# MohamedAbou-Taleb/Iterative-Linear-Quadratic-Regulator

Hardware: AMD Instinct MI355X
Metric: iLQR iterations/sec (batch=4096, T=200, n=4 m=1); backward-pass HBM GB/s (higher is better)
Workload: dtype f32

## Files before the change

### iterative-linear-quadratic-regulator_amd/csrc/backward_fused16.hpp

```cpp
#pragma once

namespace ilqr {

template <typename T, int TPW, bool PK> struct FusedCfg;
template <> struct FusedCfg<float, 16, false> { static constexpr int P = 8, RU = 8; };
#ifndef ILQR_PK_RU
#define ILQR_PK_RU 5
#endif
#ifndef ILQR_PK_PAD
#define ILQR_PK_PAD 0
#endif
template <> struct FusedCfg<float, 16, true> { static constexpr int P = 4, RU = ILQR_PK_RU; };
template <> struct FusedCfg<double, 16, false> { static constexpr int P = 4, RU = 4; };
template <> struct FusedCfg<float, 4, false> { static constexpr int P = 3, RU = 4; };
template <> struct FusedCfg<double, 4, false> { static constexpr int P = 3, RU = 3; };

template <int NU> constexpr int fused_tl() { return NU == 2 ? 68 : 52; }
template <bool PK, int NU> constexpr int fused_unit_scalars() { return (PK ? 128 : 64) * fused_tl<NU>() + (PK ? 64 * ILQR_PK_PAD : 0); }
template <typename T, int TPW, bool PK, int NU> constexpr int fused_ru() { return (PK && NU == 2 && FusedCfg<T, TPW, PK>::RU > 4) ? 4 : FusedCfg<T, TPW, PK>::RU; }
template <typename T, int TPW, bool PK, int NU = 1> constexpr int fused_lds_bytes() {
    return fused_ru<T, TPW, PK, NU>() * fused_unit_scalars<PK, NU>() * (int)sizeof(T) + (fused_ru<T, TPW, PK, NU>() + 4 + 32 + 4) * 4;
}
static_assert(fused_lds_bytes<float, 16, true, 1>() <= 160 * 1024 && fused_lds_bytes<float, 16, true, 2>() <= 160 * 1024 &&
              fused_lds_bytes<float, 16, false, 2>() <= 160 * 1024 && fused_lds_bytes<double, 16, false, 2>() <= 160 * 1024, "LDS ring exceeds a CU");
template <typename T, int TPW, bool PK> constexpr int fused_threads() { return 64 * (TPW / 4 + FusedCfg<T, TPW, PK>::P); }

template <typename T, int NU> struct FusedStep;
template <> struct FusedStep<float, 1> {
    using Tile = TileQ;
    static ILQR_DEV void load(Tile& t, const float* tp, int i, int j, int l16) {
        const float4 s = *reinterpret_cast<const float4*>(tp + 4 * j);
        const float4 v = *reinterpret_cast<const float4*>(tp + 32 + 4 * j);
        t.skj[0] = s.x; t.skj[1] = s.y; t.skj[2] = s.z; t.skj[3] = s.w;
        t.vj[0] = v.x; t.vj[1] = v.y; t.vj[2] = v.z; t.vj[3] = v.w;
        t.a = tp[l16];
        t.lxx = tp[16 + l16];
        t.c = tp[32 + l16];
    }
    static ILQR_DEV void step(const Tile& c, const LaneConst<float>& lc, int i, int j, float& V, float& vx, float& out, bool& pd) {
        RawTileQ none;
        const i32x4 srd = {0, 0, 0, 0};
        const TileOffsets off = {0, 0, 0};
        float Kj, kff;
        tile16_step_f32<false>(c, lc, V, vx, Kj, kff, pd, none, srd, off, 0);
        out = (i == 0) ? Kj : kff;
    }
    static ILQR_DEV void step_box(const Tile& c, const LaneConst<float>& lc, int i, int j, float u, float lo, float hi,
                                  float& V, float& vx, float& out, bool& pd) {
        RawTileQ none;
        const i32x4 srd = {0, 0, 0, 0};
        const TileOffsets off = {0, 0, 0};
        float Kj, kff;
        tile16_step_f32<false, true>(c, lc, V, vx, Kj, kff, pd, none, srd, off, 0, u, lo, hi);
        out = (i == 0) ? Kj : kff;
    }
};
template <> struct FusedStep<double, 1> {
    using Tile = Tile16<double>;
    static ILQR_DEV void load(Tile& t, const double* tp, int i, int j, int l16) { tile16_load_lds(t, tp, i, j, l16); }
    static ILQR_DEV void step(const Tile& c, const LaneConst<double>& lc, int i, int j, double& V, double& vx, double& out, bool& pd) {
        double Kj, kff;
        tile16_step<double, false>(c, lc, 0.0, V, vx, Kj, kff, pd);
        out = (i == 0) ? Kj : kff;
    }
    static ILQR_DEV void step_box(const Tile& c, const LaneConst<double>& lc, int i, int j, double u, double lo, double hi,
                                  double& V, double& vx, double& out, bool& pd) {
        double Kj, kff;
        tile16_step<double, false, true>(c, lc, 0.0, V, vx, Kj, kff, pd, u, lo, hi);
        out = (i == 0) ? Kj : kff;
    }
};
template <> struct FusedStep<float, 2> {
    using Tile = TileQ2;
    static ILQR_DEV void load(Tile& t, const float* tp, int i, int j, int l16) { tileq2_load_lds(t, tp, i, j, l16); }
    static ILQR_DEV void step(const Tile& c, const LaneConst<float>& lc, int i, int j, float& V, float& vx, float& out, bool& pd) {
        const GainSel sel = GainSel::of(i, j);
        tile16m2_step_f32(c, lc, sel, V, vx, out, pd);
    }
};
template <typename T> struct FusedStep<T, 2> {
    using Tile = Tile16M2<T>;
    using V4 = typename Vec4<T>::type;
    static ILQR_DEV void load(Tile& t, const T* tp, int i, int j, int l16) {
        const V4 si = *reinterpret_cast<const V4*>(tp + 4 * i);
        const V4 sj = *reinterpret_cast<const V4*>(tp + 4 * j);
        const V4 g0 = *reinterpret_cast<const V4*>(tp + 32 + 8 * j);
        const V4 g1 = *reinterpret_cast<const V4*>(tp + 36 + 8 * j);
        t.ski[0] = si.x; t.ski[1] = si.y; t.ski[2] = si.z; t.ski[3] = si.w;
        t.skj[0] = sj.x; t.skj[1] = sj.y; t.skj[2] = sj.z; t.skj[3] = sj.w;
        t.gj[0] = g0.x; t.gj[1] = g0.y; t.gj[2] = g0.z; t.gj[3] = g0.w;
        t.gj[4] = g1.x; t.gj[5] = g1.y; t.gj[6] = g1.z; t.gj[7] = g1.w;
        const T* gi = tp + 32 + 8 * i;
        t.gi[0] = gi[0]; t.gi[1] = gi[1]; t.gi[3] = gi[3]; t.gi[4] = gi[4];
        t.lxx = tp[16 + l16];
    }
    static ILQR_DEV void step(const Tile& c, const LaneConst<T>& lc, int i, int j, T& V, T& vx, T& out, bool& pd) {
        T K0, K1, k0, k1;
        tile16m2_step<T, false>(c, lc.m0, lc.m1, T(0), V, vx, K0, K1, k0, k1, pd);
        out = (i == 0) ? K0 : ((i == 1) ? K1 : ((j == 0) ? k0 : k1));
    }
};

ILQR_DEV void compiler_fence() { asm volatile("" ::: "memory"); }
ILQR_DEV int lds_peek(const int* p) { return __hip_atomic_load(p, __ATOMIC_RELAXED, __HIP_MEMORY_SCOPE_WORKGROUP); }
ILQR_DEV void lds_poke(int* p, int v) { __hip_atomic_store(p, v, __ATOMIC_RELAXED, __HIP_MEMORY_SCOPE_WORKGROUP); }

template <typename T, typename Dyn, int INTEG, int TPW, bool PK, bool BOX, bool HET> struct FusedRoles {
    static constexpr int NX = Dyn::NX, NU = Dyn::NU;
    static_assert(!BOX || (NU == 1 && fused_tl<1>() > kTile16), "control limits: n_u = 1, u_t in the tile's padding");
    static_assert((NU == 1 && NX >= 2 && NX <= 4) || (NX == 4 && NU == 2), "the fused sweep serves the DPP tiles: n_u = 1, or (4, 2)");
    static_assert(TPW == 16 || TPW == 4, "16 or 4 trajectories per workgroup");
    static_assert(!PK || (sizeof(T) == 4 && TPW == 16 && INTEG != ILQR_INT_BACKWARD_EULER), "pair producers: fp32, 16-trajectory workgroups, explicit integrators");
    using Cfg = FusedCfg<T, TPW, PK>;
    static constexpr int P = Cfg::P, RU = fused_ru<T, TPW, PK, NU>(), TL = fused_tl<NU>();
    static constexpr int NV = (NU == 2 ? kTile16M2 : kTile16) / 4;
    static constexpr int NSW = TPW / 4;
    static constexpr int UT = PK ? 128 : 64;
    static constexpr int US = UT / TPW;
    static constexpr int UNIT = fused_unit_scalars<PK, NU>();
    static constexpr int PS = 2 * TL + ILQR_PK_PAD;
    static constexpr int R = gain_record(NX, NU);
    using PL = ParamLayout<Dyn::NSYS, NX, NU>;
    using V4 = typename Vec4<T>::type;
    static ILQR_DEV constexpr int tile_off(int r, int tl) { return PK ? ((r / 2) * TPW + tl) * PS + (r % 2) * TL : (r * TPW + tl) * TL; }
    static ILQR_DEV constexpr int step_off(int r) { return PK ? (r / 2) * TPW * PS + (r % 2) * TL : r * TPW * TL; }

    struct Lds {
        T* ring;
        int* ready;
        int* done;
        int* s_slot;
        int* s_stat;
    };
    static ILQR_DEV Lds carve(unsigned char* base) {
        Lds L;
        L.ring = reinterpret_cast<T*>(base);
        L.ready = reinterpret_cast<int*>(base + (size_t)RU * UNIT * sizeof(T));
        L.done = L.ready + RU;
        L.s_slot = L.done + 4;
        L.s_stat = L.s_slot + 16;
        return L;
    }

    static ILQR_DEV void head(const KArgs<T>& a, const Lds& L, int b0, int lane, bool do_select, bool count) {
        bool still = false;
        if (lane < 16) {
            const int b = b0 + lane;
            int slot = 0, st = -1;
            if (lane < TPW && b < a.B) {
                if (do_select) {
                    still = select_candidates(a, b, true, slot, st);
                } else {
                    st = a.status[b];
                    slot = a.cur_slot[b];
                }
                a.cur_slot[b] = traj_active(st) ? 0 : slot;
            }
            L.s_slot[lane] = slot;
            L.s_stat[lane] = st;
        } else if (lane < 16 + RU + 4) {
            L.ready[lane - 16] = 0;
        }
        if (do_select && count) {
            const unsigned long long m = __ballot(still);
            if (lane == 0 && m) atomicAdd(&a.counters[a.counter_idx], (int)__popcll(m));
            if (blockIdx.x == 0 && lane == 0) a.counters[(a.counter_idx + 1) % kCounterRing] = 0;
        }
    }
    static ILQR_DEV bool any_active(const Lds& L) {
        bool any = false;
#pragma unroll
        for (int q = 0; q < 16; ++q) any = any || traj_active(L.s_stat[q]);
        return any;
    }

    static ILQR_DEV void sweep(const KArgs<T>& a, const Lds& L, int b0, int wave, int lane, ClockProbe& cp) {
        const size_t B = a.B;
        const int N = a.N;
        const int tid = threadIdx.x;
        (void)tid;
        __builtin_amdgcn_s_setprio(2);
        const int l16 = lane & 15, i = l16 >> 2, j = l16 & 3;
        const int tl = 4 * wave + (lane >> 4);
        const int gidx = b0 + tl;
        const bool valid = gidx < a.B;
        const int b = valid ? gidx : a.B - 1;
        const int st = L.s_stat[tl];
        const bool act = valid && traj_active(st);
        const int slot = act ? L.s_slot[tl] : 0;
        T ph[HET ? PL::TOTAL : 1];
        if constexpr (HET) {
#pragma unroll
            for (int q = 0; q < PL::TOTAL; ++q) ph[q] = a.params[q];
            load_row<PL::Q>(ph, a.rows, B, b);
        }
        const T* __restrict__ pp = HET ? ph : a.params;
        T xN[NX];
        vec_load<T, NX>(a.X + vec_at(B, N + 1, NX, slot, N, b), xN);
        if (act && slot != 0 && l16 == 0) vec_store<T, NX>(a.X + vec_at(B, N + 1, NX, 0, N, b), xN);
        T V = T(0), vx = T(0);
        {
            T g[NX], H[NX][NX];
            Cost<T, Dyn>::l_f_x(pp, xN, g);
            Cost<T, Dyn>::l_f_xx(pp, xN, H);
#pragma unroll
            for (int ii = 0; ii < NX; ++ii) {
                if (j == ii) vx = g[ii];
#pragma unroll
                for (int jj = 0; jj < NX; ++jj)
                    if (i == ii && j == jj) V = H[ii][jj];
            }
        }
        const unsigned gain_bytes = (unsigned)((size_t)N * B * R * sizeof(T));
        const __amdgpu_buffer_rsrc_t rgain = make_rsrc(a.gains, gain_bytes);
        const int rstride = (int)(B * R * sizeof(T));
        constexpr bool DROP = sizeof(T) == 4 || ILQR_DROP_ALL;
        const bool storer = act && (NU == 1 ? ((i == 0 && j < NX) || l16 == 4) : (i < 2 || (i == 2 && j < 2)));
        const int rec_slot = NU == 1 ? (i == 0 ? j : NX) : (i < 2 ? 4 * i + j : 8 + j);
        const int rec_off = (storer || !DROP) ? (int)((b * R + rec_slot) * sizeof(T)) : 0x7ffffff0;
        LaneConst<T> lc;
        lc.m0 = T(j == 0);
        lc.m1 = T(j == 1);
        lc.tr_byte = 4 * ((lane & 48) | (j << 2) | i);
        bool all_pd = true;
        using FS = FusedStep<T, NU>;
        const T blo = BOX ? a.u_lo[0] : T(0), bhi = BOX ? a.u_hi[0] : T(0);
        typename FS::Tile tq[2];
        T uq[2] = {T(0), T(0)};
        auto load = [&](int q, const T* tp) {
            FS::load(tq[q], tp, i, j, l16);
            if constexpr (BOX) uq[q] = tp[kTile16];
        };
        int goff = (N - 1) * rstride;
        auto unit_base = [&](int k) -> const T* { return L.ring + (size_t)(k % RU) * UNIT + tile_off(0, tl); };
        constexpr auto step_off = [](int r) { return PK ? (r / 2) * TPW * PS + (r % 2) * TL : r * TPW * TL; };
        auto one_step = [&](int q) {
            T out;
            bool pd;
            if constexpr (BOX) FS::step_box(tq[q], lc, i, j, uq[q], blo, bhi, V, vx, out, pd);
            else FS::step(tq[q], lc, i, j, V, vx, out, pd);
            all_pd = all_pd && pd;
            if (DROP || storer) buf_store1(rgain, rec_off, uniform(goff), out);
            goff -= rstride;
        };
#ifdef ILQR_FUSED_STAMPS
        const long long st_t0 = __builtin_readcyclecounter();
        long long st_spin = 0;
#endif
        while (lds_peek(&L.ready[0]) < 1) __builtin_amdgcn_s_sleep(1);
        compiler_fence();
#ifdef ILQR_FUSED_STAMPS
        const long long st_first = __builtin_readcyclecounter();
#endif
        load(0, unit_base(0));
        const int n_full = N / US, rem = N % US;
        for (int k = 0; k < n_full; ++k) {
            const T* ub = unit_base(k);
            const bool more = (k + 1) * US < N;
            int flag = 0;
#pragma unroll
            for (int r = 0; r < US; ++r) {
                if (r == US - 2 && more) flag = lds_peek(&L.ready[(k + 1) % RU]);
                if (r < US - 1) {
                    load((r + 1) & 1, ub + step_off(r + 1));
                } else if (more) {
#ifdef ILQR_FUSED_STAMPS
                    const long long w0 = __builtin_readcyclecounter();
#endif
                    while (flag < k + 2) {
                        __builtin_amdgcn_s_sleep(1);
                        flag = lds_peek(&L.ready[(k + 1) % RU]);
                    }
                    compiler_fence();
#ifdef ILQR_FUSED_STAMPS
                    st_spin += __builtin_readcyclecounter() - w0;
#endif
                    load(0, unit_base(k + 1));
                }
                one_step(r & 1);
            }
            compiler_fence();
            if (lane == 0) lds_poke(&L.done[wave], k + 1);
        }
        if (rem) {
            const T* ub = unit_base(n_full);
#pragma unroll
            for (int r = 0; r < US - 1; ++r) {
                if (r < rem) {
                    if (r + 1 < rem) load((r + 1) & 1, ub + step_off(r + 1));
                    one_step(r & 1);
                }
            }
        }
#ifdef ILQR_FUSED_STAMPS
        if (a.probe && blockIdx.x == 7 && tid == 0) {
            a.probe[5] = st_first - st_t0;
            a.probe[6] = st_spin;
            a.probe[7] = __builtin_readcyclecounter() - st_first;
        }
#endif
        cp.stop(a.probe, 0);
        if (act && l16 == 0 && !all_pd) a.status[b] = st | ILQR_TRAJ_FLAG_NON_PD;
    }

    static ILQR_DEV void produce(const KArgs<T>& a_, const Lds& L, int b0, int pw, int lane) {
        struct { int B; T dt; T* X; T* U; const T* params; const T* rows; } a = {a_.B, a_.dt, a_.X, a_.U, a_.params, a_.rows};
        const size_t B = a.B;
        const int N = a_.N;
        const int n_units = (N + US - 1) / US;
        if constexpr (PK) {
        using T2 = pair_f32;
        using Dyn2 = typename Dyn::template rebind<T2>;
        const int tl = lane % TPW, r2 = lane / TPW;
        const int gidx = b0 + tl;
        const bool valid = gidx < a.B;
        const int b = valid ? gidx : a.B - 1;
        const bool actb = valid && traj_active(L.s_stat[tl]);
        const int slot = actb ? L.s_slot[tl] : 0;
        const bool move = actb && slot != 0;
        T pl[PL::TOTAL];
#pragma unroll
        for (int q = 0; q < PL::TOTAL; ++q) pl[q] = a.params[q];
        if constexpr (HET) load_row<PL::Q>(pl, a.rows, B, b);
        const SplatParams p{pl};
        const T2 dt2 = a.dt;
        for (int k = pw; k < n_units; k += P) {
            const int ta = N - 1 - k * US - 2 * r2, tb = ta - 1;
            const bool ina = ta >= 0, inb = tb >= 0;
            const int tta = ina ? ta : 0, ttb = inb ? tb : 0;
            T xa[NX], ua[NU], xb[NX], ub[NU];
            vec_load<T, NX>(a.X + vec_at(B, N + 1, NX, slot, tta, b), xa);
            vec_load<T, NU>(a.U + vec_at(B, N, NU, slot, tta, b), ua);
            vec_load<T, NX>(a.X + vec_at(B, N + 1, NX, slot, ttb, b), xb);
            vec_load<T, NU>(a.U + vec_at(B, N, NU, slot, ttb, b), ub);
            if (move && ina) {
                vec_store<T, NX>(a.X + vec_at(B, N + 1, NX, 0, tta, b), xa);
                vec_store<T, NU>(a.U + vec_at(B, N, NU, 0, tta, b), ua);
            }
            if (move && inb) {
                vec_store<T, NX>(a.X + vec_at(B, N + 1, NX, 0, ttb, b), xb);
                vec_store<T, NU>(a.U + vec_at(B, N, NU, 0, ttb, b), ub);
            }
            T2 x[NX], u[NU], xn[NX], fx[NX][NX], fu[NX][NU];
#pragma unroll
            for (int q = 0; q < NX; ++q) { x[q].x = xa[q]; x[q].y = xb[q]; }
#pragma unroll
            for (int q = 0; q < NU; ++q) { u[q].x = ua[q]; u[q].y = ub[q]; }
            Stepper<T2, Dyn2>::step_jac(INTEG, p, dt2, x, u, xn, fx, fu);
            T2 gxn[NX], gu1[NU], lxxn[NX][NX], luxn[NU][NX], luu[NU][NU];
            Cost<T2, Dyn2>::grad(p, dt2, x, u, gxn, gu1);
            Cost<T2, Dyn2>::hess(p, dt2, x, u, lxxn, luxn, luu);
            V4 tile_a[NV], tile_b[NV];
            tile16_fill<T, NX, NU>([](T2 v) { return v.x; }, fx, fu, gxn, gu1, lxxn, luxn, luu, tile_a);
            tile16_fill<T, NX, NU>([](T2 v) { return v.y; }, fx, fu, gxn, gu1, lxxn, luxn, luu, tile_b);
            if (k >= RU) {
                const int need = k - RU + 1;
                auto slowest = [&]() {
                    int m = lds_peek(&L.done[0]);
#pragma unroll
                    for (int q = 1; q < NSW; ++q) m = min(m, lds_peek(&L.done[q]));
                    return m;
                };
                while (slowest() < need) __builtin_amdgcn_s_sleep(2);
            }
            compiler_fence();
            V4* dst = reinterpret_cast<V4*>(L.ring + (size_t)(k % RU) * UNIT + tile_off(2 * r2, tl));
            if (ina) {
#pragma unroll
                for (int q = 0; q < NV; ++q) dst[q] = tile_a[q];
            }
            if (inb) {
#pragma unroll
                for (int q = 0; q < NV; ++q) dst[TL / 4 + q] = tile_b[q];
            }
            if constexpr (BOX) {
                T* dt_ = reinterpret_cast<T*>(dst);
                if (ina) dt_[kTile16] = ua[0];
                if (inb) dt_[TL + kTile16] = ub[0];
            }
            compiler_fence();
            if (lane == 0) lds_poke(&L.ready[k % RU], k + 1);
        }
        } else {
        const int tl = lane % TPW, r = lane / TPW;
        const int gidx = b0 + tl;
        const bool valid = gidx < a.B;
        const int b = valid ? gidx : a.B - 1;
        const bool actb = valid && traj_active(L.s_stat[tl]);
        const int slot = actb ? L.s_slot[tl] : 0;
        const bool move = actb && slot != 0;
        T p[PL::TOTAL];
#pragma unroll
        for (int q = 0; q < PL::TOTAL; ++q) p[q] = a.params[q];
        if constexpr (HET) load_row<PL::Q>(p, a.rows, B, b);
        for (int k = pw; k < n_units; k += P) {
            const int t = N - 1 - k * US - r;
            const bool inr = t >= 0;
            const int tt = inr ? t : 0;
            T x[NX], u[NU];
            vec_load<T, NX>(a.X + vec_at(B, N + 1, NX, slot, tt, b), x);
            vec_load<T, NU>(a.U + vec_at(B, N, NU, slot, tt, b), u);
            if (move && inr) {
                vec_store<T, NX>(a.X + vec_at(B, N + 1, NX, 0, tt, b), x);
                vec_store<T, NU>(a.U + vec_at(B, N, NU, 0, tt, b), u);
            }
            T xn[NX], fx[NX][NX], fu[NX][NU];
            Stepper<T, Dyn>::step_jac(INTEG, p, a.dt, x, u, xn, fx, fu);
            V4 tile[NV];
            tile16_pack<T, Dyn>(p, a.dt, x, u, fx, fu, tile);
            if (k >= RU) {
                const int need = k - RU + 1;
                auto slowest = [&]() {
                    int m = lds_peek(&L.done[0]);
#pragma unroll
                    for (int q = 1; q < NSW; ++q) m = min(m, lds_peek(&L.done[q]));
                    return m;
                };
                while (slowest() < need) __builtin_amdgcn_s_sleep(2);
            }
            compiler_fence();
            if (inr) {
                constexpr int NQ = NV * (int)sizeof(V4) / 16;
                vec_u4 w[NQ];
                __builtin_memcpy(w, tile, sizeof(V4) * NV);
                vec_u4* dst = reinterpret_cast<vec_u4*>(L.ring + (size_t)(k % RU) * UNIT + tile_off(r, tl));
#pragma unroll
                for (int q = 0; q < NQ; ++q) dst[q] = w[q];
                if constexpr (BOX) reinterpret_cast<T*>(dst)[kTile16] = u[0];
            }
            compiler_fence();
            if (lane == 0) lds_poke(&L.ready[k % RU], k + 1);
        }
        }
    }
};

template <typename T, typename Dyn, int INTEG, int TPW, bool PK, bool BOX = false>
struct FusedWG : FusedRoles<T, Dyn, INTEG, TPW, PK, BOX, false> {};
template <typename T, typename Dyn, int INTEG, int TPW, bool PK, bool BOX = false>
struct FusedWGHet : FusedRoles<T, Dyn, INTEG, TPW, PK, BOX, true> {};

template <typename T, typename Dyn, int INTEG, int TPW, bool PK, bool BOX = false, bool HET = false>
__global__ void __launch_bounds__((fused_threads<T, TPW, PK>())) backward_fused16_kernel(KArgs<T> a) {
    using W = std::conditional_t<HET, FusedWGHet<T, Dyn, INTEG, TPW, PK, BOX>, FusedWG<T, Dyn, INTEG, TPW, PK, BOX>>;
    extern __shared__ __attribute__((aligned(16))) unsigned char fused_lds[];
    const typename W::Lds L = W::carve(fused_lds);
    const int tid = threadIdx.x, wave = tid >> 6, lane = tid & 63;
    const int b0 = blockIdx.x * TPW;
    ClockProbe cp;
    cp.start();
    if (wave == 0) W::head(a, L, b0, lane, a.fuse_select != 0, true);
    __syncthreads();
    if (!W::any_active(L)) return;
    if (wave < W::NSW) W::sweep(a, L, b0, wave, lane, cp);
    else W::produce(a, L, b0, wave - W::NSW, lane);
}

}
```

### iterative-linear-quadratic-regulator_amd/csrc/solver.hpp

```cpp
#pragma once
#include <hip/hip_runtime.h>
#include <hip/hip_ext.h>

#include <algorithm>
#include <cmath>
#include <cstdlib>
#include <cstdint>
#include <cstring>
#include <string>
#include <vector>

#include "kernels_wave.hpp"
#include "backward_mfma16.hpp"
#include "forward_mfma16.hpp"

namespace ilqr {

struct SolverBase {
    ilqr_config cfg{};
    std::string err;
    virtual ~SolverBase() {}
    virtual int sync() = 0;
    virtual int set_problem(const void* x0, const void* U) = 0;
    virtual int set(int field, const void* src, size_t bytes) = 0;
    virtual int get(int field, void* dst, size_t bytes) = 0;
    virtual int initial_rollout() = 0;
    virtual int linearize() = 0;
    virtual int backward() = 0;
    virtual int forward(const double* alphas, int n) = 0;
    virtual int select() = 0;
    virtual int iterate(int n) = 0;
    virtual int flush() = 0;
    virtual int solve(int32_t* iters, void* cost) = 0;
    virtual int backward_pass(const void* X, const void* U, void* Uff, void* K) = 0;
    virtual int backward_tensors(const void* lin, const void* term, void* Uff, void* K) = 0;
    virtual int forward_pass(const void* x0, double alpha, const void* X, const void* U, const void* Uff,
                             const void* K, void* Xn, void* Un, void* cost) = 0;
    virtual int eval_points(int integ, int npts, const void* x, const void* u, void** outs) = 0;
    virtual int mpc_reset(const void* x0, const void* U) = 0;
    virtual int mpc_rearm(const void* x0, const void* U) = 0;
    virtual int mpc_run(int n_steps, void* u_out, void* x_out, void* cost_out) = 0;
    virtual int status_reduce(void* dev_out4) = 0;
    virtual int probe_dump(long long* dst, size_t n) = 0;
    virtual int debug_set_stream(void* s) = 0;
    virtual int timing_enable(int on) = 0;
    virtual int timing_reset() = 0;
    virtual int timing_get(double* ms, int64_t* launches) = 0;
    virtual int algorithmic_bytes(double* bytes) = 0;
    virtual int set_control_limits(const double* u_min, const double* u_max) = 0;
    virtual int set_batch_params(int which, const double* rows, int row_len) = 0;
};

int system_dims(int system, int n_x, int n_u);
int param_count(int system, int n_x, int n_u);
int n_sys_params_abi(int system, int n_x, int n_u);
SolverBase* make_solver_f32(const ilqr_config& cfg, std::string& err, int* status);
SolverBase* make_solver_f64(const ilqr_config& cfg, std::string& err, int* status);
bool supported_f32(int system, int n_x, int n_u);
bool supported_f64(int system, int n_x, int n_u);

constexpr size_t kDescriptorMax = 0x7ffffff0ull;

#define ILQR_HIPCHK(expr)                                                                      \
    do {                                                                                       \
        hipError_t e_ = (expr);                                                                \
        if (e_ != hipSuccess) {                                                                \
            this->err = std::string(#expr) + ": " + hipGetErrorString(e_);                     \
            return ILQR_ERR_HIP;                                                               \
        }                                                                                      \
    } while (0)

struct LaunchEvents { hipEvent_t a = nullptr, b = nullptr; };
inline LaunchEvents& launch_events() { static thread_local LaunchEvents e; return e; }
#define ILQR_LAUNCH(kern, grid, block, lds, stream, ...)                                                     \
    do {                                                                                                     \
        LaunchEvents& le_ = launch_events();                                                                 \
        hipExtLaunchKernelGGL(kern, grid, block, lds, stream, le_.a, le_.b, 0, __VA_ARGS__);                 \
        le_ = LaunchEvents();                                                                                \
    } while (0)

template <typename T> struct Ops {
    void (*linearize[5])(const KArgs<T>&, hipStream_t) = {};
    void (*backward)(const KArgs<T>&, hipStream_t) = nullptr;
    void (*forward[5])(const KArgs<T>&, hipStream_t) = {};
    void (*fused[5])(const KArgs<T>&, hipStream_t) = {};
    void (*persist[5])(const KArgs<T>&, const PArgs<T>&, hipStream_t) = {};
    bool persist_any_batch[5] = {};
    bool persist_big = false;
    void (*eval)(const EvalArgs<T>&, hipStream_t) = nullptr;
    void (*mpc_advance)(const MpcArgs<T>&, hipStream_t) = nullptr;
    int n_dev_params = 0;
    int n_sys_dev = 0;
    int lin_stride = 0;
    bool tile16 = false;
    int tile_scalars = 0;
    bool lin_aos = false;
    bool canonical = false;
    bool const_lin = false;
    bool (*sweep_reads_sparse)(T mu) = nullptr;
    void (*linearize_box[5])(const KArgs<T>&, hipStream_t) = {};
    void (*backward_box)(const KArgs<T>&, hipStream_t) = nullptr;
    void (*forward_box[5])(const KArgs<T>&, hipStream_t) = {};
    bool fused_box = false;
    bool het = false;
    bool persist_het[5] = {};
};

template <typename T, int NX, int NU, typename = void> struct has_fwd_in { static constexpr bool value = false; };
template <typename T, int NX, int NU> struct has_fwd_in<T, NX, NU, decltype((void)sizeof(FwdIn<T, NX, NU>))> {
    static constexpr bool value = true;
};

#ifndef ILQR_RING_INTEG_MASK
#define ILQR_RING_INTEG_MASK 0x1f
#endif
#ifndef ILQR_FUSE_INTEG_MASK
#define ILQR_FUSE_INTEG_MASK 0x1f
#endif
inline int persist_small_max() {
    static const int v = getenv("ILQR_FUSED_SMALL_MAX") ? atoi(getenv("ILQR_FUSED_SMALL_MAX")) : 1024;
    return v;
}
#ifndef ILQR_PERSIST_INTEG_MASK
#define ILQR_PERSIST_INTEG_MASK 0x1f
#endif
#ifndef ILQR_NO_PAIR_PRODUCERS
#define ILQR_NO_PAIR_PRODUCERS 0
#endif
template <typename Dyn, typename = void> struct has_rebind { static constexpr bool value = false; };
template <typename Dyn> struct has_rebind<Dyn, std::void_t<typename Dyn::template rebind<float>>> { static constexpr bool value = true; };

template <typename T, typename Dyn, int I, int TPW, bool PK, bool BX, bool HT> constexpr auto fused_kernel() {
    if constexpr (HT) return backward_fused16_kernel<T, Dyn, I, TPW, PK, BX, true>;
    else return backward_fused16_kernel<T, Dyn, I, TPW, PK, BX>;
}
template <typename T, typename Dyn, int I, bool BX, bool HT = false>
void launch_fused_kernel(const KArgs<T>& a, hipStream_t s) {
    constexpr bool CAN_PK = sizeof(T) == 4 && I != ILQR_INT_BACKWARD_EULER && has_rebind<Dyn>::value && !ILQR_NO_PAIR_PRODUCERS;
    static const bool ok = [] {
        bool r = hipFuncSetAttribute((const void*)fused_kernel<T, Dyn, I, 16, false, BX, HT>(),
                                     hipFuncAttributeMaxDynamicSharedMemorySize, fused_lds_bytes<T, 16, false, Dyn::NU>()) == hipSuccess;
        r = r && hipFuncSetAttribute((const void*)fused_kernel<T, Dyn, I, 4, false, BX, HT>(),
                                     hipFuncAttributeMaxDynamicSharedMemorySize, fused_lds_bytes<T, 4, false, Dyn::NU>()) == hipSuccess;
        if constexpr (CAN_PK)
            r = r && hipFuncSetAttribute((const void*)fused_kernel<T, Dyn, I, 16, true, BX, HT>(),
                                         hipFuncAttributeMaxDynamicSharedMemorySize, fused_lds_bytes<T, 16, true, Dyn::NU>()) == hipSuccess;
        (void)hipGetLastError();
        return r;
    }();
    (void)ok;
    static const int force = getenv("ILQR_FUSED_TPW") ? atoi(getenv("ILQR_FUSED_TPW")) : 0;
    static const int small_max = getenv("ILQR_FUSED_SMALL_MAX") ? atoi(getenv("ILQR_FUSED_SMALL_MAX")) : 1024;
    static const bool no_pk = getenv("ILQR_FUSED_PAIRS") == nullptr;
    const bool small = force ? force == 4 : a.B <= small_max;
    if (small) {
        ILQR_LAUNCH((fused_kernel<T, Dyn, I, 4, false, BX, HT>()), dim3((a.B + 3) / 4), dim3(fused_threads<T, 4, false>()),
                    (fused_lds_bytes<T, 4, false, Dyn::NU>()), s, a);
        return;
    }
    if constexpr (CAN_PK) {
        if (!no_pk) {
            ILQR_LAUNCH((fused_kernel<T, Dyn, I, 16, true, BX, HT>()), dim3((a.B + 15) / 16), dim3(fused_threads<T, 16, true>()),
                        (fused_lds_bytes<T, 16, true, Dyn::NU>()), s, a);
            return;
        }
    }
    ILQR_LAUNCH((fused_kernel<T, Dyn, I, 16, false, BX, HT>()), dim3((a.B + 15) / 16), dim3(fused_threads<T, 16, false>()),
                (fused_lds_bytes<T, 16, false, Dyn::NU>()), s, a);
}

template <typename T, typename Dyn, int I, int TPW, bool PK, bool BX, bool HT> constexpr auto persist_kernel() {
    if constexpr (HT) return ilqr_persistent_kernel<T, Dyn, I, TPW, PK, BX, true>;
    else return ilqr_persistent_kernel<T, Dyn, I, TPW, PK, BX>;
}
template <typename T, typename Dyn, int I, bool BX, bool HT = false>
void launch_persist_kernel(const KArgs<T>& a, const PArgs<T>& pa, hipStream_t s) {
    constexpr bool BIG = I != ILQR_INT_BACKWARD_EULER && has_rebind<Dyn>::value && !ILQR_NO_PAIR_PRODUCERS;
    static const bool ok = [] {
        bool r = hipFuncSetAttribute((const void*)persist_kernel<T, Dyn, I, 4, false, BX, HT>(),
                                     hipFuncAttributeMaxDynamicSharedMemorySize, fused_lds_bytes<T, 4, false, Dyn::NU>()) == hipSuccess;
        if constexpr (BIG)
            r = r && hipFuncSetAttribute((const void*)persist_kernel<T, Dyn, I, 16, true, BX, HT>(),
                                         hipFuncAttributeMaxDynamicSharedMemorySize, fused_lds_bytes<T, 16, true, Dyn::NU>()) == hipSuccess;
        (void)hipGetLastError();
        return r;
    }();
    (void)ok;
    if constexpr (BIG) {
        if (a.B > persist_small_max()) {
            ILQR_LAUNCH((persist_kernel<T, Dyn, I, 16, true, BX, HT>()), dim3((a.B + 15) / 16), dim3(fused_threads<T, 16, true>()),
                        (fused_lds_bytes<T, 16, true, Dyn::NU>()), s, a, pa);
            return;
        }
    }
    ILQR_LAUNCH((persist_kernel<T, Dyn, I, 4, false, BX, HT>()), dim3((a.B + 3) / 4), dim3(fused_threads<T, 4, false>()),
                (fused_lds_bytes<T, 4, false, Dyn::NU>()), s, a, pa);
}

template <typename Dyn> constexpr bool box_system() {
    return Dyn::ID == ILQR_SYS_PENDULUM || Dyn::ID == ILQR_SYS_UA_DOUBLE_PENDULUM || Dyn::ID == ILQR_SYS_DOUBLE_PENDULUM;
}
#ifndef ILQR_PERSIST_HET_INTEG_MASK
#define ILQR_PERSIST_HET_INTEG_MASK 0x1f
#endif

template <typename T, typename Dyn, bool TILE, int INTEG> void set_integrator_ops(Ops<T>& o) {
    constexpr bool SMALL = all_integrators<Dyn>::value;
    constexpr bool FUSED_BOX = box_system<Dyn>() && Dyn::NU == 1;
    if constexpr (TILE && FUSED_BOX) o.fused_box = true;
    constexpr bool HETS = box_system<Dyn>();
    if constexpr (HETS) o.het = true;
    constexpr int I = (SMALL || INTEG == ILQR_INT_DISCRETE) ? INTEG : ILQR_INT_EULER;
    o.linearize[INTEG] = [](const KArgs<T>& a, hipStream_t s) {
        const size_t total = (size_t)a.B * (a.N + 1);
        constexpr int TPB = TILE ? 64 : 256;
        if constexpr (HETS) {
            if (a.het) {
                ILQR_LAUNCH((linearize_kernel<T, Dyn, TILE, I, true>), dim3((unsigned)((total + TPB - 1) / TPB)), dim3(TPB), 0, s, a);
                return;
            }
        }
        ILQR_LAUNCH((linearize_kernel<T, Dyn, TILE, I>), dim3((unsigned)((total + TPB - 1) / TPB)), dim3(TPB), 0, s, a);
    };
    if constexpr (TILE && ((ILQR_FUSE_INTEG_MASK >> I) & 1)) {
        o.fused[INTEG] = [](const KArgs<T>& a, hipStream_t s) {
            if constexpr (FUSED_BOX) {
                if (a.box && a.het) { launch_fused_kernel<T, Dyn, I, true, true>(a, s); return; }
                if (a.box) { launch_fused_kernel<T, Dyn, I, true>(a, s); return; }
            }
            if constexpr (HETS) {
                if (a.het) { launch_fused_kernel<T, Dyn, I, false, true>(a, s); return; }
            }
            launch_fused_kernel<T, Dyn, I, false>(a, s);
        };
    }
    if constexpr (TILE && sizeof(T) == 4 && ((ILQR_FUSE_INTEG_MASK >> I) & 1) && has_fwd_in<T, Dyn::NX, Dyn::NU>::value &&
                  ((ILQR_RING_INTEG_MASK >> I) & 1) && ((ILQR_PERSIST_INTEG_MASK >> I) & 1)) {
        constexpr bool BIG = I != ILQR_INT_BACKWARD_EULER && has_rebind<Dyn>::value && !ILQR_NO_PAIR_PRODUCERS;
        o.persist_big = o.persist_big || BIG;
        constexpr bool PHET = HETS && ((ILQR_PERSIST_HET_INTEG_MASK >> I) & 1);
        o.persist_het[INTEG] = PHET;
        o.persist[INTEG] = [](const KArgs<T>& a, const PArgs<T>& pa, hipStream_t s) {
            if constexpr (FUSED_BOX && PHET) {
                if (a.box && a.het) { launch_persist_kernel<T, Dyn, I, true, true>(a, pa, s); return; }
            }
            if constexpr (FUSED_BOX) {
                if (a.box) { launch_persist_kernel<T, Dyn, I, true>(a, pa, s); return; }
            }
            if constexpr (PHET) {
                if (a.het) { launch_persist_kernel<T, Dyn, I, false, true>(a, pa, s); return; }
            }
            launch_persist_kernel<T, Dyn, I, false>(a, pa, s);
        };
        o.persist_any_batch[INTEG] = BIG;
    }
    o.forward[INTEG] = [](const KArgs<T>& a, hipStream_t s) {
        const dim3 grid((a.B + 63) / 64, a.n_pass), block(64);
        if constexpr (has_fwd_in<T, Dyn::NX, Dyn::NU>::value && ((ILQR_RING_INTEG_MASK >> I) & 1)) {
            static const bool plain = getenv("ILQR_FORWARD_PLAIN") != nullptr;
            const size_t bytes_x = (size_t)a.n_slots * (a.N + 1) * Dyn::NX * a.B * sizeof(T);
            const size_t bytes_g = (size_t)a.N * a.B * gain_record(Dyn::NX, Dyn::NU) * sizeof(T);
            const bool fits = std::max(bytes_x, bytes_g) <= kDescriptorMax;
            if (fits && !plain) {
                if constexpr (HETS) {
                    if (a.het) { ILQR_LAUNCH((forward_ring_kernel_het<T, Dyn, I>), grid, block, 0, s, a); return; }
                }
                ILQR_LAUNCH((forward_ring_kernel<T, Dyn, I>), grid, block, 0, s, a);
                return;
            }
        }
        if constexpr (HETS) {
            if (a.het) { ILQR_LAUNCH((forward_kernel_het<T, Dyn, I>), grid, block, 0, s, a); return; }
        }
        ILQR_LAUNCH((forward_kernel<T, Dyn, I>), grid, block, 0, s, a);
    };
    if constexpr (box_system<Dyn>()) {
        o.linearize_box[INTEG] = [](const KArgs<T>& a, hipStream_t s) {
            const size_t total = (size_t)a.B * (a.N + 1);
            if (a.het) {
                ILQR_LAUNCH((linearize_kernel<T, Dyn, false, I, true>), dim3((unsigned)((total + 255) / 256)), dim3(256), 0, s, a);
                return;
            }
            ILQR_LAUNCH((linearize_kernel<T, Dyn, false, I>), dim3((unsigned)((total + 255) / 256)), dim3(256), 0, s, a);
        };
        o.forward_box[INTEG] = [](const KArgs<T>& a, hipStream_t s) {
            const dim3 grid((a.B + 63) / 64, a.n_pass), block(64);
            if constexpr (has_fwd_in<T, Dyn::NX, Dyn::NU>::value && ((ILQR_RING_INTEG_MASK >> I) & 1)) {
                static const bool plain = getenv("ILQR_FORWARD_PLAIN") != nullptr;
                const size_t bytes_x = (size_t)a.n_slots * (a.N + 1) * Dyn::NX * a.B * sizeof(T);
                const size_t bytes_g = (size_t)a.N * a.B * gain_record(Dyn::NX, Dyn::NU) * sizeof(T);
                if (std::max(bytes_x, bytes_g) <= kDescriptorMax && !plain) {
                    if (a.het) { ILQR_LAUNCH((forward_ring_kernel_box_het<T, Dyn, I>), grid, block, 0, s, a); return; }
                    ILQR_LAUNCH((forward_ring_kernel_box<T, Dyn, I>), grid, block, 0, s, a);
                    return;
                }
            }
            if (a.het) { ILQR_LAUNCH((forward_kernel_box_het<T, Dyn, I>), grid, block, 0, s, a); return; }
            ILQR_LAUNCH((forward_kernel_box<T, Dyn, I>), grid, block, 0, s, a);
        };
    }
}

template <typename T, typename Dyn> Ops<T> make_ops() {
    constexpr int NX = Dyn::NX, NU = Dyn::NU;
    Ops<T> o;
    constexpr bool TILE2 = (NX == 4 && NU == 2);
    constexpr bool TILE = (NU == 1 && NX >= 2 && NX <= 4) || TILE2;
    constexpr int TSC = TILE2 ? kTile16M2 : kTile16;
    o.tile16 = TILE;
    o.canonical = true;
    o.lin_stride = TILE ? TSC : (2 * NX * NX + 2 * NX * NU + NX + NU + NU * NU);
    o.tile_scalars = TILE ? TSC : 0;
    set_integrator_ops<T, Dyn, TILE, 0>(o);
    set_integrator_ops<T, Dyn, TILE, 1>(o);
    set_integrator_ops<T, Dyn, TILE, 2>(o);
    set_integrator_ops<T, Dyn, TILE, 3>(o);
    set_integrator_ops<T, Dyn, TILE, 4>(o);
    if constexpr (TILE2) {
        o.backward = [](const KArgs<T>& a, hipStream_t s) {
            static const bool pinned = [] {
                bool ok = hipFuncSetAttribute((const void*)backward_tile16m2_kernel<T, false>,
                                              hipFuncAttributeMaxDynamicSharedMemorySize, kTile16PinLds) == hipSuccess;
                ok = ok && hipFuncSetAttribute((const void*)backward_tile16m2_kernel<T, true>,
                                               hipFuncAttributeMaxDynamicSharedMemorySize, kTile16PinLds) == hipSuccess;
                (void)hipGetLastError();
                return ok && getenv("ILQR_BACKWARD_NO_PIN") == nullptr;
            }();
            const dim3 grid((a.B + 15) / 16), block(256);
            const size_t lds = pinned ? kTile16PinLds : 0;
            if (a.mu != T(0)) ILQR_LAUNCH((backward_tile16m2_kernel<T, true>), grid, block, lds, s, a);
            else ILQR_LAUNCH((backward_tile16m2_kernel<T, false>), grid, block, lds, s, a);
        };
    } else if constexpr (TILE) {
        o.backward = [](const KArgs<T>& a, hipStream_t s) {
            static const bool lds_ring = getenv("ILQR_BACKWARD_LDS_RING") != nullptr;
            const bool fits = (size_t)a.N * a.B * kTile16 * sizeof(T) <= kDescriptorMax &&
                              (size_t)a.N * a.B * gain_record(NX, 1) * sizeof(T) <= kDescriptorMax;
            if (lds_ring || !fits) {
                const dim3 grid((a.B + 3) / 4), block(64);
                if (a.mu != T(0)) ILQR_LAUNCH((backward_tile16_lds_kernel<T, true, NX>), grid, block, 0, s, a);
                else ILQR_LAUNCH((backward_tile16_lds_kernel<T, false, NX>), grid, block, 0, s, a);
                return;
            }
            static const bool pinned = [] {
                bool ok = hipFuncSetAttribute((const void*)backward_tile16_kernel<T, false, NX>,
                                              hipFuncAttributeMaxDynamicSharedMemorySize, kTile16PinLds) == hipSuccess;
                ok = ok && hipFuncSetAttribute((const void*)backward_tile16_kernel<T, true, NX>,
                                               hipFuncAttributeMaxDynamicSharedMemorySize, kTile16PinLds) == hipSuccess;
                (void)hipGetLastError();
                return ok && getenv("ILQR_BACKWARD_NO_PIN") == nullptr;
            }();
            const dim3 grid((a.B + 15) / 16), block(256);
            const size_t lds = pinned ? kTile16PinLds : 0;
            if (a.mu != T(0)) ILQR_LAUNCH((backward_tile16_kernel<T, true, NX>), grid, block, lds, s, a);
            else ILQR_LAUNCH((backward_tile16_kernel<T, false, NX>), grid, block, lds, s, a);
        };
    } else {
        o.backward = [](const KArgs<T>& a, hipStream_t s) {
            ILQR_LAUNCH((backward_lane_kernel<T, NX, NU>), dim3((a.B + 63) / 64), dim3(64), 0, s, a);
        };
    }
    if constexpr (box_system<Dyn>()) {
        o.backward_box = [](const KArgs<T>& a, hipStream_t s) {
            ILQR_LAUNCH((backward_box_kernel<T, NX, NU>), dim3((a.B + 63) / 64), dim3(64), 0, s, a);
        };
    }
    o.eval = [](const EvalArgs<T>& a, hipStream_t s) {
        ILQR_LAUNCH((eval_points_kernel<T, Dyn>), dim3((a.npts + 63) / 64), dim3(64), 0, s, a);
    };
    o.mpc_advance = [](const MpcArgs<T>& a, hipStream_t s) {
        if constexpr (box_system<Dyn>()) {
            if (a.plant_rows) { ILQR_LAUNCH((mpc_advance_kernel<T, Dyn, true>), dim3((a.B + 63) / 64), dim3(64, kMpcChunks), 0, s, a); return; }
        }
        ILQR_LAUNCH((mpc_advance_kernel<T, Dyn>), dim3((a.B + 63) / 64), dim3(64, kMpcChunks), 0, s, a);
    };
    o.n_dev_params = ParamLayout<Dyn::NSYS, NX, NU>::TOTAL;
    o.n_sys_dev = Dyn::NSYS;
    return o;
}

template <typename T, int NX, int NU> Ops<T> make_ops_wave() {
    using Dyn = Linear<T, NX, NU>;
    Ops<T> o;
    o.lin_aos = true;
    o.const_lin = true;
    o.lin_stride = 2 * NX * NX + 2 * NX * NU + NX + NU + NU * NU;
    for (int k = 0; k < 5; ++k) {
        o.linearize[k] = [](const KArgs<T>& a, hipStream_t s) {
            if (a.lin_sparse) {
                KArgs<T> w = a;
                w.t_first = a.N - 1;
                LaunchEvents le = launch_events();
                launch_events() = LaunchEvents{le.a, nullptr};
                ILQR_LAUNCH((linearize_grad_dense_kernel<T, NX, NU>), dim3((unsigned)(((size_t)a.B * a.N + 255) / 256)), dim3(256), 0, s, a);
                launch_events() = LaunchEvents{nullptr, le.b};
                ILQR_LAUNCH((linearize_wave_kernel<T, NX, NU>), dim3((unsigned)((size_t)a.B * 2)), dim3(64), 0, s, w);
                return;
            }
            ILQR_LAUNCH((linearize_wave_kernel<T, NX, NU>), dim3((unsigned)((size_t)a.B * (a.N + 1))), dim3(64), 0, s, a);
        };
    }
    for (int k = 0; k < 5; ++k) {
        o.forward[k] = [](const KArgs<T>& a, hipStream_t s) {
            static const bool plain = getenv("ILQR_FORWARD_PLAIN") != nullptr;
            if (plain) {
                if (a.integ == ILQR_INT_DISCRETE)
                    ILQR_LAUNCH((forward_kernel<T, Dyn, ILQR_INT_DISCRETE>), dim3((a.B + 63) / 64, a.n_pass), dim3(64), 0, s, a);
                else
                    ILQR_LAUNCH((forward_kernel<T, Dyn, ILQR_INT_EULER>), dim3((a.B + 63) / 64, a.n_pass), dim3(64), 0, s, a);
                return;
            }
            if constexpr (NX == 16 && NU == 8) {
                static const bool wave = getenv("ILQR_FORWARD_WAVE") != nullptr;
                const size_t bytes_x = (size_t)a.n_slots * (a.N + 1) * NX * a.B * sizeof(T);
                const size_t bytes_g = (size_t)a.N * a.B * gain_record(NX, NU) * sizeof(T);
                if (!wave && a.n_pass <= 16 && std::max(bytes_x, bytes_g) <= kDescriptorMax) {
                    ILQR_LAUNCH((forward_mfma16_kernel<T>), dim3(a.B), dim3(64), 0, s, a);
                    return;
                }
            }
            ILQR_LAUNCH((forward_wave_kernel<T, NX, NU>), dim3(a.B, a.n_pass), dim3(64), 0, s, a);
        };
    }
    if constexpr (NX == 16 && NU == 8) {
        o.sweep_reads_sparse = [](T mu) {
            return mu == T(0) && getenv("ILQR_BACKWARD_WAVE_LDS") == nullptr && getenv("ILQR_MFMA16_GENERAL") == nullptr;
        };
    }
    o.backward = [](const KArgs<T>& a, hipStream_t s) {
        if constexpr (NX == 16 && NU == 8) {
            static const bool lds_form = getenv("ILQR_BACKWARD_WAVE_LDS") != nullptr;
            if (a.mu == T(0) && !lds_form) {
                static const bool general = getenv("ILQR_MFMA16_GENERAL") != nullptr;
                if (a.const_lin && !general) ILQR_LAUNCH((backward_mfma16_kernel<T, true>), dim3(a.B), dim3(64), 0, s, a);
                else ILQR_LAUNCH((backward_mfma16_kernel<T, false>), dim3(a.B), dim3(64), 0, s, a);
                return;
            }
        }
        ILQR_LAUNCH((backward_wave_kernel<T, NX, NU>), dim3(a.B), dim3(64), 0, s, a);
    };
    o.eval = [](const EvalArgs<T>& a, hipStream_t s) {
        ILQR_LAUNCH((eval_points_kernel<T, Dyn>), dim3((a.npts + 63) / 64), dim3(64), 0, s, a);
    };
    o.mpc_advance = [](const MpcArgs<T>& a, hipStream_t s) {
        ILQR_LAUNCH((mpc_advance_kernel<T, Dyn>), dim3((a.B + 63) / 64), dim3(64, kMpcChunks), 0, s, a);
    };
    o.n_dev_params = ParamLayout<Dyn::NSYS, NX, NU>::TOTAL;
    o.n_sys_dev = Dyn::NSYS;
    return o;
}

template <typename T> bool find_ops(int system, int nx, int nu, Ops<T>* out);

inline std::vector<double> build_device_params(int system, int nx, int nu, const double* p) {
    std::vector<double> d;
    const double* q = p;
// ... 1096 lines not shown
```

Measured before the change: 29.32 million.

## Let sweep waves self-produce the first ring units and enable pair producers by default

In the pair-producer fused backward kernel with a single control input, the sweep waves now compute the first two ring units themselves using the scalar producer path (one lane per trajectory and step), instead of spinning until the producer waves fill them. Producers start at unit two, so the startup latency before the sweep can begin shrinks. The scalar producer code is factored into shared helpers. The launcher also turns on the pair-producer kernel by default, where it previously needed an env var, so the default path for large batches changes. The risk is extra register pressure in the sweep waves and a different default kernel variant.

```diff
diff --git a/iterative-linear-quadratic-regulator_amd/csrc/backward_fused16.hpp b/iterative-linear-quadratic-regulator_amd/csrc/backward_fused16.hpp
--- a/iterative-linear-quadratic-regulator_amd/csrc/backward_fused16.hpp
+++ b/iterative-linear-quadratic-regulator_amd/csrc/backward_fused16.hpp
@@ -119,6 +119,8 @@
     static constexpr int US = UT / TPW;
     static constexpr int UNIT = fused_unit_scalars<PK, NU>();
     static constexpr int PS = 2 * TL + ILQR_PK_PAD;
+    static constexpr int SELF_UNITS = (PK && NU == 1) ? 2 : 0;
+    static_assert(!SELF_UNITS || 64 == 4 * SELF_UNITS * US, "SELF: a sweep wave's 64 lanes = its 4 trajectories x the first units' steps");
     static constexpr int R = gain_record(NX, NU);
     using PL = ParamLayout<Dyn::NSYS, NX, NU>;
     using V4 = typename Vec4<T>::type;
@@ -174,6 +176,7 @@
         return any;
     }
 
+    template <int SELF = 0>
     static ILQR_DEV void sweep(const KArgs<T>& a, const Lds& L, int b0, int wave, int lane, ClockProbe& cp) {
         const size_t B = a.B;
         const int N = a.N;
@@ -247,8 +250,20 @@
         const long long st_t0 = __builtin_readcyclecounter();
         long long st_spin = 0;
 #endif
-        while (lds_peek(&L.ready[0]) < 1) __builtin_amdgcn_s_sleep(1);
-        compiler_fence();
+        if constexpr (SELF > 0) {
+            const int stl = 4 * wave + (lane & 3), r = lane >> 2;
+            const ScalarLane s = scalar_lane(a, L, b0, stl);
+            const int t = N - 1 - r;
+            const bool inr = t >= 0;
+            V4 tile[NV];
+            T u0;
+            scalar_point(a, s, N, inr ? t : 0, inr, tile, u0);
+            if (inr) scalar_put(L, r / US, r % US, stl, tile, u0);
+            compiler_fence();
+        } else {
+            while (lds_peek(&L.ready[0]) < 1) __builtin_amdgcn_s_sleep(1);
+            compiler_fence();
+        }
 #ifdef ILQR_FUSED_STAMPS
         const long long st_first = __builtin_readcyclecounter();
 #endif
@@ -267,7 +282,7 @@
 #ifdef ILQR_FUSED_STAMPS
                     const long long w0 = __builtin_readcyclecounter();
 #endif
-                    while (flag < k + 2) {
+                    while (k + 1 >= SELF && flag < k + 2) {
                         __builtin_amdgcn_s_sleep(1);
                         flag = lds_peek(&L.ready[(k + 1) % RU]);
                     }
@@ -303,6 +318,7 @@
         if (act && l16 == 0 && !all_pd) a.status[b] = st | ILQR_TRAJ_FLAG_NON_PD;
     }
 
+    template <int SELF = 0>
     static ILQR_DEV void produce(const KArgs<T>& a_, const Lds& L, int b0, int pw, int lane) {
         struct { int B; T dt; T* X; T* U; const T* params; const T* rows; } a = {a_.B, a_.dt, a_.X, a_.U, a_.params, a_.rows};
         const size_t B = a.B;
@@ -324,7 +340,7 @@
         if constexpr (HET) load_row<PL::Q>(pl, a.rows, B, b);
         const SplatParams p{pl};
         const T2 dt2 = a.dt;
-        for (int k = pw; k < n_units; k += P) {
+        for (int k = SELF + pw; k < n_units; k += P) {
             const int ta = N - 1 - k * US - 2 * r2, tb = ta - 1;
             const bool ina = ta >= 0, inb = tb >= 0;
             const int tta = ina ? ta : 0, ttb = inb ? tb : 0;
@@ -383,31 +399,13 @@
         }
         } else {
         const int tl = lane % TPW, r = lane / TPW;
-        const int gidx = b0 + tl;
-        const bool valid = gidx < a.B;
-        const int b = valid ? gidx : a.B - 1;
-        const bool actb = valid && traj_active(L.s_stat[tl]);
-        const int slot = actb ? L.s_slot[tl] : 0;
-        const bool move = actb && slot != 0;
-        T p[PL::TOTAL];
-#pragma unroll
-        for (int q = 0; q < PL::TOTAL; ++q) p[q] = a.params[q];
-        if constexpr (HET) load_row<PL::Q>(p, a.rows, B, b);
+        const ScalarLane s = scalar_lane(a, L, b0, tl);
         for (int k = pw; k < n_units; k += P) {
             const int t = N - 1 - k * US - r;
             const bool inr = t >= 0;
-            const int tt = inr ? t : 0;
-            T x[NX], u[NU];
-            vec_load<T, NX>(a.X + vec_at(B, N + 1, NX, slot, tt, b), x);
-            vec_load<T, NU>(a.U + vec_at(B, N, NU, slot, tt, b), u);
-            if (move && inr) {
-                vec_store<T, NX>(a.X + vec_at(B, N + 1, NX, 0, tt, b), x);
-                vec_store<T, NU>(a.U + vec_at(B, N, NU, 0, tt, b), u);
-            }
-            T xn[NX], fx[NX][NX], fu[NX][NU];
-            Stepper<T, Dyn>::step_jac(INTEG, p, a.dt, x, u, xn, fx, fu);
             V4 tile[NV];
-            tile16_pack<T, Dyn>(p, a.dt, x, u, fx, fu, tile);
+            T u0;
+            scalar_point(a, s, N, inr ? t : 0, inr, tile, u0);
             if (k >= RU) {
                 const int need = k - RU + 1;
                 auto slowest = [&]() {
@@ -419,19 +417,53 @@
                 while (slowest() < need) __builtin_amdgcn_s_sleep(2);
             }
             compiler_fence();
-            if (inr) {
-                constexpr int NQ = NV * (int)sizeof(V4) / 16;
-                vec_u4 w[NQ];
-                __builtin_memcpy(w, tile, sizeof(V4) * NV);
-                vec_u4* dst = reinterpret_cast<vec_u4*>(L.ring + (size_t)(k % RU) * UNIT + tile_off(r, tl));
-#pragma unroll
-                for (int q = 0; q < NQ; ++q) dst[q] = w[q];
-                if constexpr (BOX) reinterpret_cast<T*>(dst)[kTile16] = u[0];
-            }
+            if (inr) scalar_put(L, k, r, tl, tile, u0);
             compiler_fence();
             if (lane == 0) lds_poke(&L.ready[k % RU], k + 1);
         }
         }
+    }
+
+    struct ScalarLane {
+        int b, slot;
+        bool move;
+        T p[PL::TOTAL];
+    };
+    template <typename A> static ILQR_DEV ScalarLane scalar_lane(const A& a, const Lds& L, int b0, int tl) {
+        ScalarLane s;
+        const int gidx = b0 + tl;
+        const bool valid = gidx < a.B;
+        s.b = valid ? gidx : a.B - 1;
+        const bool actb = valid && traj_active(L.s_stat[tl]);
+        s.slot = actb ? L.s_slot[tl] : 0;
+        s.move = actb && s.slot != 0;
+#pragma unroll
+        for (int q = 0; q < PL::TOTAL; ++q) s.p[q] = a.params[q];
+        if constexpr (HET) load_row<PL::Q>(s.p, a.rows, (size_t)a.B, s.b);
+        return s;
+    }
+    template <typename A> static ILQR_DEV void scalar_point(const A& a, const ScalarLane& s, int N, int tt, bool inr, V4* tile, T& u0) {
+        const size_t B = a.B;
+        T x[NX], u[NU];
+        vec_load<T, NX>(a.X + vec_at(B, N + 1, NX, s.slot, tt, s.b), x);
+        vec_load<T, NU>(a.U + vec_at(B, N, NU, s.slot, tt, s.b), u);
+        if (s.move && inr) {
+            vec_store<T, NX>(a.X + vec_at(B, N + 1, NX, 0, tt, s.b), x);
+            vec_store<T, NU>(a.U + vec_at(B, N, NU, 0, tt, s.b), u);
+        }
+        T xn[NX], fx[NX][NX], fu[NX][NU];
+        Stepper<T, Dyn>::step_jac(INTEG, s.p, a.dt, x, u, xn, fx, fu);
+        tile16_pack<T, Dyn>(s.p, a.dt, x, u, fx, fu, tile);
+        u0 = u[0];
+    }
+    static ILQR_DEV void scalar_put(const Lds& L, int k, int r, int tl, const V4* tile, T u0) {
+        constexpr int NQ = NV * (int)sizeof(V4) / 16;
+        vec_u4 w[NQ];
+        __builtin_memcpy(w, tile, sizeof(V4) * NV);
+        vec_u4* dst = reinterpret_cast<vec_u4*>(L.ring + (size_t)(k % RU) * UNIT + tile_off(r, tl));
+#pragma unroll
+        for (int q = 0; q < NQ; ++q) dst[q] = w[q];
+        if constexpr (BOX) reinterpret_cast<T*>(dst)[kTile16] = u0;
     }
 };
 
@@ -452,8 +484,8 @@
     if (wave == 0) W::head(a, L, b0, lane, a.fuse_select != 0, true);
     __syncthreads();
     if (!W::any_active(L)) return;
-    if (wave < W::NSW) W::sweep(a, L, b0, wave, lane, cp);
-    else W::produce(a, L, b0, wave - W::NSW, lane);
+    if (wave < W::NSW) W::template sweep<W::SELF_UNITS>(a, L, b0, wave, lane, cp);
+    else W::template produce<W::SELF_UNITS>(a, L, b0, wave - W::NSW, lane);
 }
 
 }
diff --git a/iterative-linear-quadratic-regulator_amd/csrc/solver.hpp b/iterative-linear-quadratic-regulator_amd/csrc/solver.hpp
--- a/iterative-linear-quadratic-regulator_amd/csrc/solver.hpp
+++ b/iterative-linear-quadratic-regulator_amd/csrc/solver.hpp
@@ -151,7 +151,10 @@
     (void)ok;
     static const int force = getenv("ILQR_FUSED_TPW") ? atoi(getenv("ILQR_FUSED_TPW")) : 0;
     static const int small_max = getenv("ILQR_FUSED_SMALL_MAX") ? atoi(getenv("ILQR_FUSED_SMALL_MAX")) : 1024;
-    static const bool no_pk = getenv("ILQR_FUSED_PAIRS") == nullptr;
+    static const bool no_pk = [] {
+        const char* e = getenv("ILQR_FUSED_PAIRS");
+        return e != nullptr && atoi(e) == 0;
+    }();
     const bool small = force ? force == 4 : a.B <= small_max;
     if (small) {
         ILQR_LAUNCH((fused_kernel<T, Dyn, I, 4, false, BX, HT>()), dim3((a.B + 3) / 4), dim3(fused_threads<T, 4, false>()),
```

Result: faster. 29.79 million (median of 6 runs) (+1.6%).
